# google/automl

Measured on AMD Instinct MI355X. Metric: images/sec EfficientDet-D0 640x640 fwd+bwd (whole job; per-GPU = value / n_gpus), higher is better.
Workload: dtype bf16; 1 GPU; efficientdet-d0 640x640 batch 128/GPU forward+backward+SGD/EMA update (BASELINE configs[2]; DP replicas of it for n_gpus>1); global_batch=128, parallelism=dp1, ranks_seen=1, param_crc32=4110976682, launch=hipGraph replay of the captured step

## Files before the change

automl_amd/csrc/fuse.hip:

```cpp
#include "rowmap_impl.h"

namespace {

constexpr int THREADS = 256;
static_assert(THREADS == ROW_THREADS, "ew_grid sizes its grids for this workgroup size");

struct FuseArgs {
  edet_tview_t in[3];
  int mode[3];
  int pad_t[3], pad_l[3];
  int nin;
  const float* wn;
  int wc;
  int act;
  int n, oh, ow, c, ldo;
  void* gin[3];
  int gbeta[3];
  int write_ds;
  const float* wraw[3];
  float* wn_out;
  int method;
};

__device__ __forceinline__ void normalise_weights(const float (&w)[3], int nin, int method, float (&wn)[3]) {
  if (method == 1) {
    for (int i = 0; i < nin; ++i) wn[i] = 1.f;
    return;
  }
  if (method == 2) {
    float m = w[0], e[3], s = 0.f;
    for (int i = 1; i < nin; ++i) m = fmaxf(m, w[i]);
    for (int i = 0; i < nin; ++i) { e[i] = expf(w[i] - m); s += e[i]; }
    for (int i = 0; i < nin; ++i) wn[i] = e[i] / s;
    return;
  }
  float r[3], s = 0.f;
  for (int i = 0; i < nin; ++i) { r[i] = fmaxf(w[i], 0.f); s += r[i]; }
  for (int i = 0; i < nin; ++i) wn[i] = r[i] / (s + 0.0001f);
}

__device__ __forceinline__ void normalise_weights_bwd(const float (&w)[3], int nin, int method, const float (&dwn)[3],
                                                      float (&dw)[3]) {
  for (int i = 0; i < 3; ++i) dw[i] = 0.f;
  if (method == 1) return;
  if (method == 2) {
    float m = w[0], p[3], s = 0.f, dot = 0.f;
    for (int i = 1; i < nin; ++i) m = fmaxf(m, w[i]);
    for (int i = 0; i < nin; ++i) { p[i] = expf(w[i] - m); s += p[i]; }
    for (int i = 0; i < nin; ++i) { p[i] /= s; dot += dwn[i] * p[i]; }
    for (int i = 0; i < nin; ++i) dw[i] = p[i] * (dwn[i] - dot);
    return;
  }
  float r[3], s = 0.0001f, dot = 0.f;
  for (int i = 0; i < nin; ++i) { r[i] = fmaxf(w[i], 0.f); s += r[i]; }
  for (int i = 0; i < nin; ++i) dot += dwn[i] * r[i];
  for (int i = 0; i < nin; ++i) {
    const float dr = dwn[i] / s - dot / (s * s);
    if (w[i] > 0.f) dw[i] = dr;
  }
}

__device__ __forceinline__ void affine8(const edet_tview_t& v, const ViewCoef& k, float x[8]) {
  if (v.scale) {
#pragma unroll
    for (int e = 0; e < 8; ++e) x[e] = fmaf(x[e], k.scale[e], k.shift[e]);
  }
}

template <typename T, bool ARGMAX>
__device__ __forceinline__ void sample_input(const FuseArgs& a, int i, const ViewCoef& k, int n, int oy,
                                             int ox, int c0, float x[8], uint32_t (&am)[2]) {
  const edet_tview_t& v = a.in[i];
  const T* base = reinterpret_cast<const T*>(v.data);
  if (a.mode[i] == EDET_RS_IDENTITY) {
    load8<T>(base + ((size_t)(n * v.h + oy) * v.w + ox) * v.ld + c0, x);
    affine8(v, k, x);
  } else if (a.mode[i] == EDET_RS_UP2) {
    int sy = a.oh == 2 * v.h ? oy >> 1 : (int)((uint32_t)(oy * v.h) / (uint32_t)a.oh);
    int sx = a.ow == 2 * v.w ? ox >> 1 : (int)((uint32_t)(ox * v.w) / (uint32_t)a.ow);
    sy = sy < v.h - 1 ? sy : v.h - 1;
    sx = sx < v.w - 1 ? sx : v.w - 1;
    load8<T>(base + ((size_t)(n * v.h + sy) * v.w + sx) * v.ld + c0, x);
    affine8(v, k, x);
  } else {
#pragma unroll
    for (int e = 0; e < 8; ++e) x[e] = -INFINITY;
    int idx[8];
#pragma unroll
    for (int e = 0; e < 8; ++e) idx[e] = 0;
    for (int ky = 0; ky < 3; ++ky) {
      const int sy = oy * 2 - a.pad_t[i] + ky;
      if (sy < 0 || sy >= v.h) continue;
      for (int kx = 0; kx < 3; ++kx) {
        const int sx = ox * 2 - a.pad_l[i] + kx;
        if (sx < 0 || sx >= v.w) continue;
        float t[8];
        load8<T>(base + ((size_t)(n * v.h + sy) * v.w + sx) * v.ld + c0, t);
        affine8(v, k, t);
        if (ARGMAX) {
#pragma unroll
          for (int e = 0; e < 8; ++e) {
            const bool gt = t[e] > x[e];
            idx[e] = gt ? ky * 3 + kx : idx[e];
            x[e] = gt ? t[e] : x[e];
          }
        } else {
#pragma unroll
          for (int e = 0; e < 8; ++e) x[e] = fmaxf(x[e], t[e]);
        }
      }
    }
    if (ARGMAX) {
      am[0] = (uint32_t)idx[0] | ((uint32_t)idx[1] << 8) | ((uint32_t)idx[2] << 16) | ((uint32_t)idx[3] << 24);
      am[1] = (uint32_t)idx[4] | ((uint32_t)idx[5] << 8) | ((uint32_t)idx[6] << 16) | ((uint32_t)idx[7] << 24);
    }
  }
}

template <typename T, bool BWD, bool PCDW>
__device__ __forceinline__ void fuse_body(const FuseArgs& a, T* __restrict__ out, const T* __restrict__ dout,
                                          T* __restrict__ ds, float* dwn, unsigned char* __restrict__ pool_argmax,
                                          float* dwn_parts) {
  const int nvec = a.c / 8;
  const int64_t total = (int64_t)a.n * a.oh * a.ow * nvec;
  const bool per_ch = a.wc > 1;
  extern __shared__ float redc[];
  float wn[3] = {0.f, 0.f, 0.f};
  if (!BWD && !per_ch && a.wn_out) {
    float w[3] = {0.f, 0.f, 0.f};
    if (a.method != 1)
      for (int i = 0; i < a.nin; ++i) w[i] = a.wraw[i][0];
    normalise_weights(w, a.nin, a.method, wn);
    if (blockIdx.x == 0 && threadIdx.x < a.nin) a.wn_out[threadIdx.x] = wn[threadIdx.x];
  } else if (!per_ch) {
    for (int i = 0; i < a.nin; ++i) wn[i] = a.wn[i];
  }
  float dw_acc[3] = {0.f, 0.f, 0.f};
  float dwc[PCDW ? 3 : 1][8];
  uint32_t q0 = blockIdx.x * blockDim.x + threadIdx.x, qstride = gridDim.x * blockDim.x;
  const int slices = PCDW ? THREADS / nvec : 1;
  if (PCDW) {
#pragma unroll
    for (int i = 0; i < 3; ++i)
#pragma unroll
      for (int e = 0; e < 8; ++e) dwc[PCDW ? i : 0][e] = 0.f;
    const int chunk = threadIdx.x % nvec, slice = threadIdx.x / nvec;
    q0 = slice < slices ? (uint32_t)((blockIdx.x * slices + slice) * nvec + chunk) : (uint32_t)total;
    qstride = (uint32_t)(gridDim.x * slices * nvec);
  }
  const uint32_t total32 = (uint32_t)total, unvec = (uint32_t)nvec, uow = (uint32_t)a.ow, uoh = (uint32_t)a.oh;
  for (uint32_t q = q0; q < total32; q += qstride) {
    uint32_t pix = q / unvec;
    const int c0 = (int)(q - pix * unvec) * 8;
    const uint32_t prow = pix / uow;
    const int ox = (int)(pix - prow * uow);
    const int n = (int)(prow / uoh);
    const int oy = (int)(prow - (uint32_t)n * uoh);
    float s[8], xi[3][8];
#pragma unroll
    for (int e = 0; e < 8; ++e) s[e] = 0.f;
    const size_t opix = (size_t)(n * a.oh + oy) * a.ow + ox;
    int plane = 0;
    for (int i = 0; i < a.nin; ++i) {
      ViewCoef k;
      view_load_coef(a.in[i], c0, k);
      uint32_t am[2];
      if (BWD && pool_argmax && a.mode[i] == EDET_RS_POOL) {
        sample_input<T, true>(a, i, k, n, oy, ox, c0, xi[i], am);
        *reinterpret_cast<uint2*>(pool_argmax + ((size_t)plane * a.n * a.oh * a.ow + opix) * a.c + c0) =
            make_uint2(am[0], am[1]);
        ++plane;
      } else {
        sample_input<T, false>(a, i, k, n, oy, ox, c0, xi[i], am);
      }
      if (per_ch) {
        float wv[8];
        loadf8(a.wn + (size_t)i * a.wc + c0, wv);
#pragma unroll
        for (int e = 0; e < 8; ++e) s[e] = fmaf(wv[e], xi[i][e], s[e]);
      } else {
#pragma unroll
        for (int e = 0; e < 8; ++e) s[e] = fmaf(wn[i], xi[i][e], s[e]);
      }
    }
    const size_t off = opix * a.ldo + c0;
    if (!BWD) {
      if (a.act == EDET_ACT_SWISH) {
#pragma unroll
        for (int e = 0; e < 8; ++e) s[e] = swishf_(s[e]);
      } else if (a.act > EDET_ACT_SWISH) {
#pragma unroll
        for (int e = 0; e < 8; ++e) s[e] = act_other_(a.act, s[e]);
      }
      store8<T>(out + off, s);
    } else {
      float d[8];
      load8<T>(dout + off, d);
      if (a.act == EDET_ACT_SWISH) {
#pragma unroll
        for (int e = 0; e < 8; ++e) d[e] *= swish_gradf_(s[e]);
      } else if (a.act > EDET_ACT_SWISH) {
#pragma unroll
        for (int e = 0; e < 8; ++e) d[e] *= act_other_grad_(a.act, s[e]);
      }
      if (a.write_ds) store8<T>(ds + off, d);
      for (int i = 0; i < a.nin; ++i) {
        if (a.gin[i]) {
          float g[8];
#pragma unroll
          for (int e = 0; e < 8; ++e) g[e] = to_f<T>(from_f<T>(d[e]));
          if (per_ch) {
            float wv[8];
            loadf8(a.wn + (size_t)i * a.wc + c0, wv);
#pragma unroll
            for (int e = 0; e < 8; ++e) g[e] *= wv[e];
          } else {
#pragma unroll
            for (int e = 0; e < 8; ++e) g[e] *= wn[i];
          }
          T* gp = reinterpret_cast<T*>(a.gin[i]) + opix * a.in[i].ld + c0;
          if (a.gbeta[i]) {
            float old[8];
            load8<T>(gp, old);
#pragma unroll
            for (int e = 0; e < 8; ++e) g[e] += old[e];
          }
          store8<T>(gp, g);
        }
      }
      for (int i = 0; i < a.nin; ++i) {
        if (per_ch) {
          if (PCDW) {
#pragma unroll
// ... 13 lines not shown
#pragma unroll
        for (int e = 0; e < 8; ++e) redc[((size_t)slice * a.nin + i) * a.c + chunk * 8 + e] = dwc[PCDW ? i : 0][e];
    }
    __syncthreads();
    for (int i = threadIdx.x; i < a.nin * a.c; i += THREADS) {
      float t = 0.f;
      for (int sl = 0; sl < slices; ++sl) t += redc[(size_t)sl * a.nin * a.c + i];
      if (dwn_parts) dwn_parts[(size_t)blockIdx.x * a.nin * a.c + i] = t;
      else dwn[i] += t;
    }
  } else if (BWD && dwn && !per_ch) {
    __shared__ float red[THREADS / 64][4];
    for (int i = 0; i < a.nin; ++i) {
      float v = dw_acc[i];
#pragma unroll
      for (int off = 32; off > 0; off >>= 1) v += __shfl_down(v, off, 64);
      if ((threadIdx.x & 63) == 0) red[threadIdx.x >> 6][i] = v;
    }
    __syncthreads();
    if (threadIdx.x < 3) {
      float t = 0.f;
      if (threadIdx.x < a.nin)
        for (int w = 0; w < THREADS / 64; ++w) t += red[w][threadIdx.x];
      if (dwn_parts) dwn_parts[(size_t)blockIdx.x * 4 + threadIdx.x] = t;
      else if (threadIdx.x < a.nin) dwn[threadIdx.x] += t;
    }
  }
}

template <typename T, bool BWD>
__global__ __launch_bounds__(THREADS) void k_fuse(const FuseArgs a, T* __restrict__ out,
                                                 const T* __restrict__ dout, T* __restrict__ ds,
                                                 float* dwn, unsigned char* __restrict__ pool_argmax,
                                                 float* dwn_parts = nullptr) {
  fuse_body<T, BWD, false>(a, out, dout, ds, dwn, pool_argmax, dwn_parts);
}
template <typename T>
__global__ __launch_bounds__(THREADS) void k_fuse_pc(const FuseArgs a, T* __restrict__ out,
                                                    const T* __restrict__ dout, T* __restrict__ ds,
                                                    float* dwn, unsigned char* __restrict__ pool_argmax,
                                                    float* dwn_parts) {
  fuse_body<T, true, true>(a, out, dout, ds, dwn, pool_argmax, dwn_parts);
}

struct FuseWBwd {
  const float* w[3];
  float* dw[3];
  int nin, method;
};
__global__ __launch_bounds__(256) void k_fuse_dwn_finish(const float* __restrict__ parts, int G, float* dwn, FuseWBwd wb) {
  __shared__ float red[256][3];
  __shared__ float tot[3];
  float t[3] = {0.f, 0.f, 0.f};
  const int per = (G + 255) / 256;
  for (int g = threadIdx.x * per; g < min(G, (threadIdx.x + 1) * per); ++g)
    for (int i = 0; i < 3; ++i) t[i] += parts[(size_t)g * 4 + i];
  for (int i = 0; i < 3; ++i) red[threadIdx.x][i] = t[i];
  __syncthreads();
  if (threadIdx.x < 3) {
    float s = 0.f;
    for (int q = 0; q < 256; ++q) s += red[q][threadIdx.x];
    dwn[threadIdx.x] += s;
    tot[threadIdx.x] = dwn[threadIdx.x];
  }
  if (wb.nin == 0 || wb.method == 1) return;
  __syncthreads();
  if (threadIdx.x == 0) {
    float w[3] = {0.f, 0.f, 0.f}, d[3] = {tot[0], tot[1], tot[2]}, dw[3];
    for (int i = 0; i < wb.nin; ++i) w[i] = wb.w[i][0];
    normalise_weights_bwd(w, wb.nin, wb.method, d, dw);
    for (int i = 0; i < wb.nin; ++i)
      if (wb.method == 2 || w[i] > 0.f) wb.dw[i][0] += dw[i];
  }
}

struct FuseInArgs {
  edet_tview_t in;
  int mode, pad_t, pad_l;
  const float* wn;
  int wc;
  int idx;
  int n, oh, ow, ldds;
  int beta;
};

template <typename T>
__global__ __launch_bounds__(THREADS) void k_fuse_bwd_input(const FuseInArgs a, const T* __restrict__ ds,
                                                           T* __restrict__ gout,
                                                           const unsigned char* __restrict__ argmax) {
  const edet_tview_t& v = a.in;
  const int nvec = v.c / 8;
  const int64_t total = (int64_t)v.n * v.h * v.w * nvec;
  const float wn = a.wc > 1 ? 0.f : a.wn[a.idx];
  const T* base = reinterpret_cast<const T*>(v.data);
  const uint32_t total32 = (uint32_t)total, unvec = (uint32_t)nvec, uw = (uint32_t)v.w, uh = (uint32_t)v.h;
  for (uint32_t q = blockIdx.x * blockDim.x + threadIdx.x; q < total32; q += gridDim.x * blockDim.x) {
    const uint32_t pix = q / unvec;
    const int c0 = (int)(q - pix * unvec) * 8;
    const uint32_t prow = pix / uw;
    const int sx = (int)(pix - prow * uw);
    const int n = (int)(prow / uh);
    const int sy = (int)(prow - (uint32_t)n * uh);
    float g[8];
#pragma unroll
    for (int e = 0; e < 8; ++e) g[e] = 0.f;
    if (a.mode == EDET_RS_IDENTITY) {
      load8<T>(ds + ((size_t)(n * a.oh + sy) * a.ow + sx) * a.ldds + c0, g);
    } else if (a.mode == EDET_RS_UP2) {
      const bool x2 = a.oh == 2 * v.h && a.ow == 2 * v.w;
      const int oy_lo = x2 ? 2 * sy : (int)(((uint32_t)(sy * a.oh) + uh - 1) / uh);
      int oy_hi = x2 ? 2 * sy + 2 : (int)(((uint32_t)((sy + 1) * a.oh) + uh - 1) / uh);
      const int ox_lo = x2 ? 2 * sx : (int)(((uint32_t)(sx * a.ow) + uw - 1) / uw);
      int ox_hi = x2 ? 2 * sx + 2 : (int)(((uint32_t)((sx + 1) * a.ow) + uw - 1) / uw);
      if (sy == v.h - 1) oy_hi = a.oh;
      if (sx == v.w - 1) ox_hi = a.ow;
      for (int oy = oy_lo; oy < oy_hi; ++oy)
        for (int ox = ox_lo; ox < ox_hi; ++ox) {
          float t[8];
          load8<T>(ds + ((size_t)(n * a.oh + oy) * a.ow + ox) * a.ldds + c0, t);
#pragma unroll
          for (int e = 0; e < 8; ++e) g[e] += t[e];
        }
    } else if (argmax) {
      for (int oy = (sy + a.pad_t - 2 + 1) / 2; oy <= (sy + a.pad_t) / 2; ++oy) {
        if (oy < 0 || oy >= a.oh) continue;
        for (int ox = (sx + a.pad_l - 2 + 1) / 2; ox <= (sx + a.pad_l) / 2; ++ox) {
          if (ox < 0 || ox >= a.ow) continue;
          const uint32_t tap = (uint32_t)((sy - (oy * 2 - a.pad_t)) * 3 + (sx - (ox * 2 - a.pad_l)));
          const size_t opix = (size_t)(n * a.oh + oy) * a.ow + ox;
          const uint2 am = *reinterpret_cast<const uint2*>(argmax + opix * v.c + c0);
          float t[8];
          load8<T>(ds + opix * a.ldds + c0, t);
#pragma unroll
          for (int e = 0; e < 8; ++e) {
            const uint32_t w = e < 4 ? am.x : am.y;
            if (((w >> (8 * (e & 3))) & 0xffu) == tap) g[e] += t[e];
          }
        }
      }
    } else {
      ViewCoef k;
      view_load_coef(v, c0, k);
      float mine[8];
      load8<T>(base + ((size_t)(n * v.h + sy) * v.w + sx) * v.ld + c0, mine);
      affine8(v, k, mine);
      for (int oy = (sy + a.pad_t - 2 + 1) / 2; oy <= (sy + a.pad_t) / 2; ++oy) {
        if (oy < 0 || oy >= a.oh) continue;
        for (int ox = (sx + a.pad_l - 2 + 1) / 2; ox <= (sx + a.pad_l) / 2; ++ox) {
          if (ox < 0 || ox >= a.ow) continue;
          bool win[8];
#pragma unroll
          for (int e = 0; e < 8; ++e) win[e] = true;
          for (int ky = 0; ky < 3; ++ky) {
            const int yy = oy * 2 - a.pad_t + ky;
            if (yy < 0 || yy >= v.h) continue;
            for (int kx = 0; kx < 3; ++kx) {
              const int xx = ox * 2 - a.pad_l + kx;
              if (xx < 0 || xx >= v.w) continue;
              if (yy == sy && xx == sx) continue;
              float t[8];
              load8<T>(base + ((size_t)(n * v.h + yy) * v.w + xx) * v.ld + c0, t);
              affine8(v, k, t);
              const bool before = (yy < sy) || (yy == sy && xx < sx);
#pragma unroll
              for (int e = 0; e < 8; ++e) {
                if (before ? (t[e] >= mine[e]) : (t[e] > mine[e])) win[e] = false;
              }
            }
          }
          float t[8];
          load8<T>(ds + ((size_t)(n * a.oh + oy) * a.ow + ox) * a.ldds + c0, t);
#pragma unroll
          for (int e = 0; e < 8; ++e)
            if (win[e]) g[e] += t[e];
        }
      }
    }
    const size_t off = ((size_t)(n * v.h + sy) * v.w + sx) * v.ld + c0;
    if (a.wc > 1) {
      float wv[8];
      loadf8(a.wn + (size_t)a.idx * a.wc + c0, wv);
#pragma unroll
      for (int e = 0; e < 8; ++e) g[e] *= wv[e];
    } else {
#pragma unroll
      for (int e = 0; e < 8; ++e) g[e] *= wn;
    }
    if (a.beta) {
      float old[8];
      load8<T>(gout + off, old);
#pragma unroll
      for (int e = 0; e < 8; ++e) g[e] += old[e];
    }
    store8<T>(gout + off, g);
  }
}

__global__ void k_fuse_weights(const float* w0, const float* w1, const float* w2, int nin, int method,
                               float* wn, int wc) {
  const int ch = blockIdx.x * blockDim.x + threadIdx.x;
  if (ch >= wc) return;
  const float* wp[3] = {w0, w1, w2};
  float w[3] = {0.f, 0.f, 0.f}, r[3];
  if (method != 1)
    for (int i = 0; i < nin; ++i) w[i] = wp[i][ch];
  normalise_weights(w, nin, method, r);
  for (int i = 0; i < nin; ++i) wn[i * wc + ch] = r[i];
}

__global__ void k_fuse_weights_bwd(const float* w0, const float* w1, const float* w2, int nin, int method,
                                   const float* dwn, float* dw0, float* dw1, float* dw2, int wc) {
  const int ch = blockIdx.x * blockDim.x + threadIdx.x;
  if (ch >= wc || method == 1) return;
  const float* wp[3] = {w0, w1, w2};
  float* dwp[3] = {dw0, dw1, dw2};
  float w[3] = {0.f, 0.f, 0.f}, d[3] = {0.f, 0.f, 0.f}, dw[3];
  for (int i = 0; i < nin; ++i) { w[i] = wp[i][ch]; d[i] = dwn[i * wc + ch]; }
  normalise_weights_bwd(w, nin, method, d, dw);
  for (int i = 0; i < nin; ++i)
    if (method == 2 || w[i] > 0.f) dwp[i][ch] += dw[i];
}

int fill_args(FuseArgs& a, const edet_tview_t* in0, const edet_tview_t* in1, const edet_tview_t* in2,
              const int* modes, int nin, const float* wn, int wc, int act, int oh, int ow, int ldo) {
  EDET_CHECK(nin >= 1 && nin <= 3 && in0 && modes && wn, "edet_fuse: bad arguments");
  EDET_CHECK(wc == 1 || wc == in0->c, "edet_fuse: wc must be 1 or the channel count (got %d)", wc);
  const edet_tview_t* ins[3] = {in0, in1, in2};
  memset(&a, 0, sizeof(a));
  a.nin = nin; a.wn = wn; a.wc = wc; a.act = act; a.oh = oh; a.ow = ow; a.ldo = ldo;
  for (int i = 0; i < nin; ++i) {
    EDET_CHECK(ins[i] && ins[i]->data, "edet_fuse: null input %d", i);
    a.in[i] = *ins[i];
    a.mode[i] = modes[i];
    EDET_CHECK(ins[i]->act == EDET_ACT_NONE && !ins[i]->gate, "edet_fuse: inputs must be affine-only views");
    EDET_CHECK(ins[i]->c == in0->c && ins[i]->n == in0->n && ins[i]->c % 8 == 0 && ins[i]->ld % 8 == 0,
               "edet_fuse: channel/batch mismatch");
    if (modes[i] == EDET_RS_IDENTITY) {
      EDET_CHECK(ins[i]->h == oh && ins[i]->w == ow, "edet_fuse: identity input %d has a different size", i);
    } else if (modes[i] == EDET_RS_UP2) {
      EDET_CHECK(ins[i]->h <= oh && ins[i]->w <= ow, "edet_fuse: upsample input %d is larger than the output", i);
    } else if (modes[i] == EDET_RS_POOL) {
      EDET_CHECK(same_out(ins[i]->h, 2) == oh && same_out(ins[i]->w, 2) == ow,
                 "Incompatible Resampling : feat shape %dx%d target_shape: %dx%d", ins[i]->h, ins[i]->w, oh, ow);
      a.pad_t[i] = same_pad_before(ins[i]->h, 3, 2);
      a.pad_l[i] = same_pad_before(ins[i]->w, 3, 2);
    } else {
      EDET_CHECK(false, "edet_fuse: bad mode %d", modes[i]);
    }
  }
  a.n = in0->n; a.c = in0->c;
  EDET_CHECK(ldo % 8 == 0 && ldo >= a.c, "edet_fuse: bad ldo");
  return 0;
}

}

extern "C" int edet_fuse_weights(const float* w0, const float* w1, const float* w2, int nin,
                                 int method, float* wn, int wc, void* stream) {
  EDET_CHECK(wn && (method == 1 || w0) && wc >= 1, "edet_fuse_weights: bad arguments");
  edet_launch(k_fuse_weights, dim3((wc + 63) / 64), dim3(64), 0, to_stream(stream), w0, w1, w2, nin, method, wn, wc);
  EDET_LAUNCH_CHECK("edet_fuse_weights");
  return 0;
}

extern "C" int edet_fuse_weights_bwd(const float* w0, const float* w1, const float* w2, int nin,
                                     int method, const float* dwn, float* dw0, float* dw1, float* dw2,
                                     int wc, void* stream) {
  if (method == 1) return 0;
  EDET_CHECK(w0 && dwn && dw0 && wc >= 1, "edet_fuse_weights_bwd: bad arguments");
  edet_launch(k_fuse_weights_bwd, dim3((wc + 63) / 64), dim3(64), 0, to_stream(stream), w0, w1, w2, nin, method, dwn, dw0, dw1, dw2, wc);
  EDET_LAUNCH_CHECK("edet_fuse_weights_bwd");
  return 0;
}

extern "C" int edet_fuse_fwd(const edet_tview_t* in0, const edet_tview_t* in1, const edet_tview_t* in2,
                             const int* modes, int nin, float* wn, int wc, int act,
                             void* out, int oh, int ow, int ldo, const float* const* wraw, int method, int dtype,
                             void* stream) {
  FuseArgs a;
  if (int rc = fill_args(a, in0, in1, in2, modes, nin, wn, wc, act, oh, ow, ldo)) return rc;
  EDET_CHECK(out, "edet_fuse_fwd: null output");
  if (wraw && wc == 1) {
    EDET_CHECK(method >= 0 && method <= 2, "edet_fuse_fwd: bad method %d", method);
    for (int i = 0; i < nin; ++i) {
      EDET_CHECK(method == 1 || wraw[i], "edet_fuse_fwd: null fusion variable %d", i);
      a.wraw[i] = wraw[i];
    }
    a.wn_out = wn;
    a.method = method;
  }
  EDET_CHECK((int64_t)a.n * oh * ow * (a.c / 8) < (1ll << 31), "edet_fuse_fwd: tensor too large for the 32-bit index arithmetic");
  const int grid = ew_grid((int64_t)a.n * oh * ow * (a.c / 8), dtype == EDET_BF16 ? reinterpret_cast<const void*>(&k_fuse<bf16_t, false>) : nullptr);
  if (dtype == EDET_BF16) edet_launch(k_fuse<bf16_t, false>, grid, dim3(THREADS), 0, to_stream(stream), a, (bf16_t*)out, nullptr, nullptr, nullptr, nullptr, nullptr);
  else if (dtype == EDET_F32) edet_launch(k_fuse<float, false>, grid, dim3(THREADS), 0, to_stream(stream), a, (float*)out, nullptr, nullptr, nullptr, nullptr, nullptr);
  else EDET_CHECK(false, "edet_fuse_fwd: bad dtype %d", dtype);
  EDET_LAUNCH_CHECK("edet_fuse_fwd");
  return 0;
}

extern "C" int edet_fuse_bwd_pre(const edet_tview_t* in0, const edet_tview_t* in1, const edet_tview_t* in2,
                                 const int* modes, int nin, const float* wn, int wc, int act,
                                 const void* dout, int oh, int ow, int ldo,
                                 void* ds, float* dwn, void* pool_argmax, void* const* gin, const int* gbeta,
                                 int write_ds, void* workspace, size_t workspace_bytes, const float* const* wraw,
                                 int method, float* const* dwraw, int dtype, void* stream) {
  FuseArgs a;
  if (int rc = fill_args(a, in0, in1, in2, modes, nin, wn, wc, act, oh, ow, ldo)) return rc;
  EDET_CHECK(dout && ds, "edet_fuse_bwd_pre: null pointer");
  a.write_ds = write_ds;
  for (int i = 0; i < nin; ++i) {
    a.gin[i] = gin ? gin[i] : nullptr;
    a.gbeta[i] = (gin && gbeta) ? gbeta[i] : 0;
    EDET_CHECK(!a.gin[i] || modes[i] == EDET_RS_IDENTITY, "edet_fuse_bwd_pre: gin[%d] given for a resampled input", i);
  }
  const bool pcdw = wc > 1 && dwn;
  EDET_CHECK(!pcdw || a.c <= 8 * THREADS, "edet_fuse_bwd_pre: per-channel fusion weights need c <= %d", 8 * THREADS);
  const size_t lds = pcdw ? (size_t)(THREADS / (a.c / 8)) * nin * a.c * sizeof(float) : 0;
  EDET_CHECK((int64_t)a.n * oh * ow * (a.c / 8) < (1ll << 31), "edet_fuse_bwd_pre: tensor too large for the 32-bit index arithmetic");
  int grid = ew_grid((int64_t)a.n * oh * ow * (a.c / 8), dtype == EDET_BF16 ? (pcdw ? reinterpret_cast<const void*>(&k_fuse_pc<bf16_t>) : reinterpret_cast<const void*>(&k_fuse<bf16_t, true>)) : nullptr, lds);
  const size_t row = pcdw ? (size_t)nin * a.c : 4;
  float* parts = (dwn && workspace && workspace_bytes >= (size_t)grid * row * sizeof(float)) ? reinterpret_cast<float*>(workspace) : nullptr;
  if (dwn && !parts) grid = 1;
  if (pcdw) {
    if (dtype == EDET_BF16) edet_launch(k_fuse_pc<bf16_t>, grid, dim3(THREADS), lds, to_stream(stream), a, nullptr, (const bf16_t*)dout, (bf16_t*)ds, dwn, (unsigned char*)pool_argmax, parts);
    else if (dtype == EDET_F32) edet_launch(k_fuse_pc<float>, grid, dim3(THREADS), lds, to_stream(stream), a, nullptr, (const float*)dout, (float*)ds, dwn, (unsigned char*)pool_argmax, parts);
    else EDET_CHECK(false, "edet_fuse_bwd_pre: bad dtype %d", dtype);
    EDET_LAUNCH_CHECK("edet_fuse_bwd_pre");
    if (parts && edet_reduce_partials2(parts, grid, (int64_t)nin * a.c, dwn, (int64_t)nin * a.c, nullptr, to_stream(stream)) != 0) return -2;
    return 0;
  }
  if (dtype == EDET_BF16) edet_launch(k_fuse<bf16_t, true>, grid, dim3(THREADS), lds, to_stream(stream), a, nullptr, (const bf16_t*)dout, (bf16_t*)ds, dwn, (unsigned char*)pool_argmax, parts);
  else if (dtype == EDET_F32) edet_launch(k_fuse<float, true>, grid, dim3(THREADS), lds, to_stream(stream), a, nullptr, (const float*)dout, (float*)ds, dwn, (unsigned char*)pool_argmax, parts);
  else EDET_CHECK(false, "edet_fuse_bwd_pre: bad dtype %d", dtype);
  if (parts) {
    FuseWBwd wb;
    memset(&wb, 0, sizeof(wb));
    if (wraw && dwraw && method != 1) {
      EDET_CHECK(method == 0 || method == 2, "edet_fuse_bwd_pre: bad method %d", method);
      for (int i = 0; i < nin; ++i) {
        EDET_CHECK(wraw[i] && dwraw[i], "edet_fuse_bwd_pre: null fusion variable %d", i);
        wb.w[i] = wraw[i];
        wb.dw[i] = dwraw[i];
      }
      wb.nin = nin;
      wb.method = method;
    }
    edet_launch(k_fuse_dwn_finish, dim3(1), dim3(256), 0, to_stream(stream), (const float*)parts, grid, dwn, wb);
  } else {
    EDET_CHECK(!(wraw && dwraw) || method == 1, "edet_fuse_bwd_pre: the fusion variables' gradient needs wc == 1 and a workspace of %zu bytes",
               (size_t)grid * 4 * sizeof(float));
  }
  EDET_LAUNCH_CHECK("edet_fuse_bwd_pre");
  return 0;
}

extern "C" int edet_fuse_bwd_input(const edet_tview_t* in, int mode, const float* wn, int wc, int idx,
                                   const void* ds, int oh, int ow, int lds_, const void* pool_argmax,
                                   void* gout, int beta, int dtype, void* stream) {
  EDET_CHECK(in && in->data && wn && ds && gout && idx >= 0 && idx < 3, "edet_fuse_bwd_input: bad arguments");
  EDET_CHECK(in->c % 8 == 0 && in->ld % 8 == 0 && lds_ % 8 == 0, "edet_fuse_bwd_input: c/ld % 8");
  EDET_CHECK(wc == 1 || wc == in->c, "edet_fuse_bwd_input: wc must be 1 or the channel count (got %d)", wc);
  FuseInArgs a;
  memset(&a, 0, sizeof(a));
  a.in = *in; a.mode = mode; a.wn = wn; a.wc = wc; a.idx = idx; a.n = in->n; a.oh = oh; a.ow = ow; a.ldds = lds_;
  a.beta = beta;
  if (mode == EDET_RS_POOL) {
    a.pad_t = same_pad_before(in->h, 3, 2);
    a.pad_l = same_pad_before(in->w, 3, 2);
  }
  EDET_CHECK((int64_t)in->n * in->h * in->w * (in->c / 8) < (1ll << 31), "edet_fuse_bwd_input: tensor too large for the 32-bit index arithmetic");
  const int grid = ew_grid((int64_t)in->n * in->h * in->w * (in->c / 8), dtype == EDET_BF16 ? reinterpret_cast<const void*>(&k_fuse_bwd_input<bf16_t>) : nullptr);
  const unsigned char* am = mode == EDET_RS_POOL ? reinterpret_cast<const unsigned char*>(pool_argmax) : nullptr;
  if (dtype == EDET_BF16) edet_launch(k_fuse_bwd_input<bf16_t>, grid, dim3(THREADS), 0, to_stream(stream), a, (const bf16_t*)ds, (bf16_t*)gout, am);
  else if (dtype == EDET_F32) edet_launch(k_fuse_bwd_input<float>, grid, dim3(THREADS), 0, to_stream(stream), a, (const float*)ds, (float*)gout, am);
  else EDET_CHECK(false, "edet_fuse_bwd_input: bad dtype %d", dtype);
  EDET_LAUNCH_CHECK("edet_fuse_bwd_input");
  return 0;
}
```

automl_amd/engine.py:

```python
import ctypes

import torch

from automl_amd import _lib
from automl_amd import netspec as netspec_lib
from automl_amd._lib import ACT_NONE, ACT_SWISH, EDET_BF16, RS_IDENTITY, RS_POOL, RS_UP2, call, ptr
from automl_amd.layer_engine import BN, LayerEngine, ParamArena, Raw, Update, View, capture_graph


class Engine(LayerEngine):

  def __init__(self, config, batch_size, image_size=None, dtype='bf16', device='cuda:0', seed=0,
               params=None, spec=None, stochastic_depth=True, arena=None):
    self.config = config
    momentum = float(config.momentum)
    adam = str(config.optimizer).lower() == 'adam'
    super().__init__(spec if spec is not None else netspec_lib.NetSpec(config), batch_size,
                     image_size if image_size is not None else config.image_size, dtype=dtype, device=device, seed=seed,
                     params=params, arena=arena, stochastic_depth=stochastic_depth,
                     update=Update('adam', momentum, self.ADAM_BETA2, self.ADAM_EPSILON) if adam else Update('sgd', momentum))
    if adam:
      self.arena.second_moment()
    self._side = None
    self.small_level_stream = True
    self._side_pending = False
    self.loss_sums = self.zbuf('loss_sums', (4,))
    self.pool_argmax = True
    self._overlap_reduce = None
    self._reduce_marks = {}
    self._comm_stream = None
    self._bucket_no = 0

  def _side_branch(self):
    if self._side is None:
      names = [n for n in self.seg_names if n.startswith('class_net/') or n.startswith('box_net/')]
      lo = min(self.offsets[n][0] for n in names)
      hi = max(self.offsets[n][0] + self.offsets[n][1] for n in names)
      self._side_range = (lo, hi)
      self._side_grads = torch.zeros(self.n_train_elems, dtype=torch.float32, device=self.device)
      self._side = self._new_branch(torch.cuda.Stream(device=self.device), self._side_grads)
    return self._side

  def _fork_join(self, main_job, side_job):
    side = self._side_branch()
    main = torch.cuda.current_stream(self.device)
    rec = _lib.recorder
    fork = torch.cuda.Event()
    fork.record(main)
    side.stream.wait_event(fork)
    if rec is not None:
      rec.stream_wait(side.stream.cuda_stream, rec.event_record(main.cuda_stream))
    try:
      self._branch = side
      with torch.cuda.stream(side.stream):
        b = side_job()
        done = torch.cuda.Event()
        done.record(side.stream)
        rec_done = rec.event_record(side.stream.cuda_stream) if rec is not None else None
      self._branch = self._main
      a = main_job()
    finally:
      self._branch = self._main
    main.wait_event(done)
    if rec is not None:
      rec.stream_wait(main.cuda_stream, rec_done)
    return a, b

  def _join_side(self):
    if self._side_pending:
      lo, hi = self._side_range
      call('edet_axpy_clear', self.grads_flat.data_ptr() + 4 * lo, self._side_grads.data_ptr() + 4 * lo, hi - lo, 1,
           self.stream)
      self._side_pending = False

  def fuse(self, key, inputs, modes, wnames, oh, ow, act=ACT_SWISH):
    c = inputs[0].raw.c
    n = inputs[0].raw.n
    nin = len(inputs)
    out = Raw(self, key, n, oh, ow, c)
    wm = self.spec.fpn.weight_method
    wc = c if (wnames and wm.startswith('channel_')) else 1
    wn = self.buf(key + ':wn', (max(4, 3 * wc),), torch.float32)
    method = (2 if wm in ('attn', 'channel_attn') else 0) if wnames else 1
    wp = [ptr(self.param(w)) for w in wnames] + [None] * (3 - len(wnames)) if wnames else [None] * 3
    wfold = wc == 1
    wraw = (ctypes.c_void_p * 3)(*wp) if wfold else None
    if not wfold:
      call('edet_fuse_weights', wp[0], wp[1], wp[2], nin, method, ptr(wn), wc, self.stream)
    tv = [v.tview() for v in inputs]
    tvp = [ctypes.byref(t) for t in tv] + [None] * (3 - nin)
    marr = (ctypes.c_int * 3)(*(list(modes) + [0] * (3 - nin)))
    fbytes = (sum(v.raw.rows for v in inputs) + out.rows) * c * self.esize
    call('edet_fuse_fwd', tvp[0], tvp[1], tvp[2], marr, nin, ptr(wn), wc, act, ptr(out.data), oh, ow, out.ld,
         wraw, method, self.dtype, self.stream, nbytes=fbytes)
    vout = View(out)
    for v in inputs:
      v.consumers += 1
    if self.training:
      ds = self.buf(key + ':ds', (n, oh, ow, out.ld), self.tdtype)
      dwn = self.zbuf(key + ':dwn', (max(4, 3 * wc),))
      npool = sum(1 for m in modes if m == RS_POOL)
      amax = self.buf(key + ':amax', (npool, n, oh, ow, c), torch.uint8) if npool and self.pool_argmax else None

      def bwd():
        assert out.grad_written, key
        tv2 = [v.tview() for v in inputs]
        tvp2 = [ctypes.byref(t) for t in tv2] + [None] * (3 - nin)
        merged = [modes[i] == RS_IDENTITY and v.raw.needs_grad for i, v in enumerate(inputs)]
        gin = (ctypes.c_void_p * 3)()
        gbeta = (ctypes.c_int * 3)()
        for i, v in enumerate(inputs):
          if merged[i]:
            gin[i] = ptr(v.raw.ensure_grad())
            gbeta[i] = 1 if v.raw.grad_written else 0
            v.raw.grad_written = True
        write_ds = 1 if any(v.raw.needs_grad and not merged[i] for i, v in enumerate(inputs)) else 0
        wgrad_folded = wfold and bool(wnames) and method != 1
        dwraw = (ctypes.c_void_p * 3)(*([ptr(self.grad(w)) for w in wnames] + [None] * (3 - len(wnames)))) if wgrad_folded else None
        call('edet_fuse_bwd_pre', tvp2[0], tvp2[1], tvp2[2], marr, nin, ptr(wn), wc, act, ptr(out.grad), oh, ow,
             out.ld, ptr(ds), ptr(dwn), ptr(amax), gin, gbeta, write_ds, *self._ws(),
             wraw if wgrad_folded else None, method, dwraw, self.dtype, self.stream,
             nbytes=fbytes + out.rows * c * self.esize)
        plane = 0
        for i, v in enumerate(inputs):
          am = None
          if modes[i] == RS_POOL and amax is not None:
            am = amax[plane].data_ptr()
            plane += 1
          if not v.raw.needs_grad or merged[i]:
            continue
          g = v.raw.ensure_grad()
          call('edet_fuse_bwd_input', ctypes.byref(tv2[i]), modes[i], ptr(wn), wc, i, ptr(ds), oh, ow, out.ld, am,
               ptr(g), 1 if v.raw.grad_written else 0, self.dtype, self.stream,
               nbytes=(out.rows + v.raw.rows) * c * self.esize,
               tag='%dx%dx%d %s' % (v.raw.h, v.raw.w, c, ('id', 'up2', 'pool')[modes[i]]))
          v.raw.grad_written = True
        if wnames and not wgrad_folded:
          gp = [ptr(self.grad(w)) for w in wnames] + [None] * (3 - len(wnames))
          call('edet_fuse_weights_bwd', wp[0], wp[1], wp[2], nin, method, ptr(dwn), gp[0], gp[1], gp[2],
               wc, self.stream)

      self.tape.append(bwd)
    return vout

  def forward(self, images, training=False, update_moving=True):
    c = self.config
    spec = self.spec
    self._begin(training, update_moving)
    if training and self.drop_masks and not torch.cuda.is_current_stream_capturing():
      self.refresh_drop_masks()
    bb = c.backbone_name
    x = self.stem(bb, images, self.act)
    reds = []
    self._reduce_marks = {}
    bucket_blocks = self._bucket_blocks() if (training and self._overlap_reduce is not None) else ()
    for b in spec.blocks:
      if b.index in bucket_blocks:
        self._reduce_marks[len(self.tape)] = bucket_blocks[b.index]
      x = self._mbconv(x, b, '%s/blocks_%d' % (bb, b.index))
      if b.index in spec.reductions:
        reds.append(x)
    all_feats = [None] + reds
    feats = list(all_feats[c.min_level:c.max_level + 1])
    wf = c.fpn_num_filters
    if training and self._overlap_reduce is not None:
      self._reduce_marks[0] = 0
      self._reduce_marks[len(self.tape)] = self._first_non_backbone_elem()
    for level in range(6, c.max_level + 1):
      f = feats[-1]
      th, tw = (f.raw.h + 1) // 2, (f.raw.w + 1) // 2
      s = 'resample_p%d' % level
      if f.raw.c != wf and getattr(c, 'conv_after_downsample', False):
        pooled = self.fuse(s + ':pool', [f], [RS_POOL], [], th, tw, act=ACT_NONE)
        feats.append(self.pw(s, pooled, s + '/conv2d/kernel', wf, bias=s + '/conv2d/bias', bn=(s + '/bn') if c.apply_bn_for_resampling else None, bias_grad=True))
        continue
      if f.raw.c != wf:
        f = self.pw(s, f, s + '/conv2d/kernel', wf, bias=s + '/conv2d/bias', bn=(s + '/bn') if c.apply_bn_for_resampling else None, bias_grad=True)
      feats.append(self.fuse(s + ':pool', [f], [RS_POOL], [], th, tw, act=ACT_NONE))
    for rep in range(c.fpn_cell_repeats):
      feats = self._fpn_cell(feats, 'fpn_cells/cell_%d' % rep)
    self.fpn_feats = feats
    na = spec.num_anchors
    nbig = sum(1 for f in feats if f.raw.h * f.raw.w > 400)
    if self.small_level_stream and self.sync_bn is None and 0 < nbig < len(feats):
      cls, box = self._heads_two_chains(feats, nbig, c.num_classes * na, 4 * na)
    else:
      cls = self._head(feats, 'class_net', 'class', c.num_classes * na)
      box = self._head(feats, 'box_net', 'box', 4 * na)
    self.cls_views, self.box_views = cls, box
    if self._cast_items and not torch.cuda.is_current_stream_capturing() and \
        (self._cast_table is None or self._cast_table[0] != list(self._cast_items)):
      self._cast_all()
    return cls, box

  def _fpn_cell(self, feats, cell_scope):
    c = self.config
    wf = c.fpn_num_filters
    fpn = self.spec.fpn
    feats = list(feats)
# ... 301 lines not shown
```

Before: 2886 images/sec.

## Add specialized BiFPN fuse fast paths and merge up2 input gradient into fused backward

Adds templated fast paths for the common BiFPN fusion patterns (identity+upsample2, identity+pool, identity+identity+pool). They batch raw vector loads ahead of the math, hoist the per-channel affine coefficients, and unroll over several grid strides. In backward, the upsampled input's gradient is now computed inside the pre-kernel by iterating over coarse pixels and summing their four fine children. This removes the separate bwd_input launch and the ds buffer write/read for that case. It also adds dedicated up2 and pool-argmax paths in the standalone input-gradient kernel, at the cost of more template instantiations and register pressure.

```diff
diff --git a/automl_amd/csrc/fuse.hip b/automl_amd/csrc/fuse.hip
--- a/automl_amd/csrc/fuse.hip
+++ b/automl_amd/csrc/fuse.hip
@@ -20,6 +20,28 @@
   const float* wraw[3];
   float* wn_out;
   int method;
+  int fast;
+};
+
+enum { FUSE_GENERIC = 0, FUSE_ID_UP2 = 1, FUSE_ID_ID_POOL = 2, FUSE_ID_POOL = 3, FUSE_ID_UP2_QUAD = 4 };
+constexpr int FUSE_DEPTH_UP2 = 2, FUSE_DEPTH_POOL = 1;
+
+template <typename T> struct Raw8;
+template <> struct Raw8<bf16_t> {
+  uint4 v;
+  __device__ __forceinline__ void load(const bf16_t* p) { v = *reinterpret_cast<const uint4*>(p); }
+  __device__ __forceinline__ void get(float x[8]) const { unpack8(v, x); }
+};
+template <> struct Raw8<float> {
+  float4 a, b;
+  __device__ __forceinline__ void load(const float* p) {
+    a = *reinterpret_cast<const float4*>(p);
+    b = *reinterpret_cast<const float4*>(p + 4);
+  }
+  __device__ __forceinline__ void get(float x[8]) const {
+    x[0] = a.x; x[1] = a.y; x[2] = a.z; x[3] = a.w;
+    x[4] = b.x; x[5] = b.y; x[6] = b.z; x[7] = b.w;
+  }
 };
 
 __device__ __forceinline__ void normalise_weights(const float (&w)[3], int nin, int method, float (&wn)[3]) {
@@ -114,6 +136,269 @@
       am[0] = (uint32_t)idx[0] | ((uint32_t)idx[1] << 8) | ((uint32_t)idx[2] << 16) | ((uint32_t)idx[3] << 24);
       am[1] = (uint32_t)idx[4] | ((uint32_t)idx[5] << 8) | ((uint32_t)idx[6] << 16) | ((uint32_t)idx[7] << 24);
     }
+  }
+}
+
+template <typename T, bool BWD, int NIN, int LAST, int UU>
+__device__ __forceinline__ void fuse_fast_trip(const FuseArgs& a, T* __restrict__ out, const T* __restrict__ dout,
+                                               T* __restrict__ ds, unsigned char* __restrict__ pool_argmax,
+                                               const float (&wn)[3], ViewCoef (&k)[NIN], bool hoisted, uint32_t q,
+                                               uint32_t qstride, float (&dw_acc)[3]) {
+  constexpr int NID = NIN - 1, NTAP = LAST == EDET_RS_POOL ? 9 : 1;
+  const uint32_t unvec = (uint32_t)(a.c / 8), uow = (uint32_t)a.ow, uoh = (uint32_t)a.oh;
+  const edet_tview_t& vl = a.in[NID];
+  int c0[UU];
+  size_t opix[UU];
+  uint32_t inside[UU];
+  Raw8<T> rid[UU][NID], rlast[UU][NTAP], rd[UU], rold[UU][NID];
+#pragma unroll
+  for (int u = 0; u < UU; ++u) {
+    const uint32_t qq = q + (uint32_t)u * qstride;
+    const uint32_t pix = qq / unvec;
+    c0[u] = (int)(qq - pix * unvec) * 8;
+    const uint32_t prow = pix / uow;
+    const int ox = (int)(pix - prow * uow);
+    const int n = (int)(prow / uoh);
+    const int oy = (int)(prow - (uint32_t)n * uoh);
+    opix[u] = (size_t)(n * a.oh + oy) * a.ow + ox;
+#pragma unroll
+    for (int i = 0; i < NID; ++i)
+      rid[u][i].load(reinterpret_cast<const T*>(a.in[i].data) + opix[u] * a.in[i].ld + c0[u]);
+    const T* base = reinterpret_cast<const T*>(vl.data);
+    inside[u] = 0;
+    if (LAST == EDET_RS_UP2) {
+      rlast[u][0].load(base + ((size_t)(n * vl.h + (oy >> 1)) * vl.w + (ox >> 1)) * vl.ld + c0[u]);
+    } else {
+#pragma unroll
+      for (int ky = 0; ky < 3; ++ky) {
+        const int sy = oy * 2 - a.pad_t[NID] + ky;
+        const int cy = min(max(sy, 0), vl.h - 1);
+#pragma unroll
+        for (int kx = 0; kx < 3; ++kx) {
+          const int sx = ox * 2 - a.pad_l[NID] + kx;
+          const int cx = min(max(sx, 0), vl.w - 1);
+          inside[u] |= (sy == cy && sx == cx) ? 1u << (ky * 3 + kx) : 0u;
+          rlast[u][NTAP == 9 ? ky * 3 + kx : 0].load(base + ((size_t)(n * vl.h + cy) * vl.w + cx) * vl.ld + c0[u]);
+        }
+      }
+    }
+    if (BWD) {
+      rd[u].load(dout + opix[u] * a.ldo + c0[u]);
+#pragma unroll
+      for (int i = 0; i < NID; ++i)
+        if (a.gin[i] && a.gbeta[i])
+          rold[u][i].load(reinterpret_cast<const T*>(a.gin[i]) + opix[u] * a.in[i].ld + c0[u]);
+    }
+  }
+#pragma unroll
+  for (int u = 0; u < UU; ++u) {
+    if (!hoisted) {
+#pragma unroll
+      for (int i = 0; i < NIN; ++i) view_load_coef(a.in[i], c0[u], k[i]);
+    }
+    float s[8], xi[NIN][8];
+#pragma unroll
+    for (int e = 0; e < 8; ++e) s[e] = 0.f;
+#pragma unroll
+    for (int i = 0; i < NID; ++i) {
+      rid[u][i].get(xi[i]);
+      affine8(a.in[i], k[i], xi[i]);
+#pragma unroll
+      for (int e = 0; e < 8; ++e) s[e] = fmaf(wn[i], xi[i][e], s[e]);
+    }
+    if (LAST == EDET_RS_UP2) {
+      rlast[u][0].get(xi[NID]);
+      affine8(vl, k[NID], xi[NID]);
+    } else {
+      int idx[8];
+#pragma unroll
+      for (int e = 0; e < 8; ++e) { xi[NID][e] = -INFINITY; idx[e] = 0; }
+#pragma unroll
+      for (int tap = 0; tap < NTAP; ++tap) {
+        float t[8];
+        rlast[u][tap].get(t);
+        affine8(vl, k[NID], t);
+        const bool in = (inside[u] >> tap) & 1u;
+#pragma unroll
+        for (int e = 0; e < 8; ++e) {
+          t[e] = in ? t[e] : -INFINITY;
+          if (BWD) {
+            const bool gt = t[e] > xi[NID][e];
+            idx[e] = gt ? tap : idx[e];
+            xi[NID][e] = gt ? t[e] : xi[NID][e];
+          } else {
+            xi[NID][e] = fmaxf(xi[NID][e], t[e]);
+          }
+        }
+      }
+      if (BWD)
+        *reinterpret_cast<uint2*>(pool_argmax + opix[u] * a.c + c0[u]) =
+            make_uint2((uint32_t)idx[0] | ((uint32_t)idx[1] << 8) | ((uint32_t)idx[2] << 16) | ((uint32_t)idx[3] << 24),
+                       (uint32_t)idx[4] | ((uint32_t)idx[5] << 8) | ((uint32_t)idx[6] << 16) | ((uint32_t)idx[7] << 24));
+    }
+#pragma unroll
+    for (int e = 0; e < 8; ++e) s[e] = fmaf(wn[NID], xi[NID][e], s[e]);
+    const size_t off = opix[u] * a.ldo + c0[u];
+    if (!BWD) {
+      if (a.act == EDET_ACT_SWISH) {
+#pragma unroll
+        for (int e = 0; e < 8; ++e) s[e] = swishf_(s[e]);
+      } else if (a.act > EDET_ACT_SWISH) {
+#pragma unroll
+        for (int e = 0; e < 8; ++e) s[e] = act_other_(a.act, s[e]);
+      }
+      store8<T>(out + off, s);
+    } else {
+      float d[8];
+      rd[u].get(d);
+      if (a.act == EDET_ACT_SWISH) {
+#pragma unroll
+        for (int e = 0; e < 8; ++e) d[e] *= swish_gradf_(s[e]);
+      } else if (a.act > EDET_ACT_SWISH) {
+#pragma unroll
+        for (int e = 0; e < 8; ++e) d[e] *= act_other_grad_(a.act, s[e]);
+      }
+      if (a.write_ds) store8<T>(ds + off, d);
+#pragma unroll
+      for (int i = 0; i < NID; ++i) {
+        if (a.gin[i]) {
+#pragma clang fp contract(off)
+          float g[8];
+#pragma unroll
+          for (int e = 0; e < 8; ++e) g[e] = to_f<T>(from_f<T>(d[e]));
+#pragma unroll
+          for (int e = 0; e < 8; ++e) g[e] *= wn[i];
+          if (a.gbeta[i]) {
+            float old[8];
+            rold[u][i].get(old);
+#pragma unroll
+            for (int e = 0; e < 8; ++e) g[e] += old[e];
+          }
+          store8<T>(reinterpret_cast<T*>(a.gin[i]) + opix[u] * a.in[i].ld + c0[u], g);
+        }
+      }
+#pragma unroll
+      for (int i = 0; i < NIN; ++i)
+#pragma unroll
+        for (int e = 0; e < 8; ++e) dw_acc[i] = fmaf(d[e], xi[i][e], dw_acc[i]);
+    }
+  }
+}
+
+template <typename T, bool BWD, int NIN, int LAST>
+__device__ __forceinline__ void fuse_fast_loop(const FuseArgs& a, T* __restrict__ out, const T* __restrict__ dout,
+                                               T* __restrict__ ds, unsigned char* __restrict__ pool_argmax,
+                                               const float (&wn)[3], uint32_t q0, uint32_t qstride, uint32_t total32,
+                                               float (&dw_acc)[3]) {
+  const uint32_t unvec = (uint32_t)(a.c / 8);
+  const bool hoisted = qstride % unvec == 0;
+  ViewCoef k[NIN];
+  if (hoisted) {
+#pragma unroll
+    for (int i = 0; i < NIN; ++i) view_load_coef(a.in[i], (int)(q0 % unvec) * 8, k[i]);
+  }
+  constexpr int DEPTH = LAST == EDET_RS_POOL ? FUSE_DEPTH_POOL : FUSE_DEPTH_UP2;
+  uint32_t q = q0;
+  for (; q + (DEPTH - 1) * qstride < total32; q += DEPTH * qstride)
+    fuse_fast_trip<T, BWD, NIN, LAST, DEPTH>(a, out, dout, ds, pool_argmax, wn, k, hoisted, q, qstride, dw_acc);
+  for (; q < total32; q += qstride)
+    fuse_fast_trip<T, BWD, NIN, LAST, 1>(a, out, dout, ds, pool_argmax, wn, k, hoisted, q, qstride, dw_acc);
+}
+
+
+template <typename T>
+__device__ __forceinline__ void fuse_up2_quad_loop(const FuseArgs& a, const T* __restrict__ dout, T* __restrict__ ds,
+                                                   const float (&wn)[3], uint32_t q0, uint32_t qstride,
+                                                   float (&dw_acc)[3]) {
+  const edet_tview_t& vc = a.in[1];
+  const uint32_t unvec = (uint32_t)(a.c / 8), uw = (uint32_t)vc.w, uh = (uint32_t)vc.h;
+  const uint32_t total32 = (uint32_t)a.n * uh * uw * unvec;
+  const bool hoisted = qstride % unvec == 0;
+  ViewCoef k[2];
+  if (hoisted) {
+#pragma unroll
+    for (int i = 0; i < 2; ++i) view_load_coef(a.in[i], (int)(q0 % unvec) * 8, k[i]);
+  }
+  const bool old0 = a.gin[0] && a.gbeta[0], old1 = a.gbeta[1] != 0;
+  for (uint32_t q = q0; q < total32; q += qstride) {
+    const uint32_t pix = q / unvec;
+    const int c0 = (int)(q - pix * unvec) * 8;
+    const uint32_t prow = pix / uw;
+    const int sx = (int)(pix - prow * uw);
+    const int n = (int)(prow / uh);
+    const int sy = (int)(prow - (uint32_t)n * uh);
+    const size_t cpix = (size_t)(n * vc.h + sy) * vc.w + sx;
+    size_t opix[4];
+    Raw8<T> rc, rid[4], rd[4], rold0[4], rold1;
+    rc.load(reinterpret_cast<const T*>(vc.data) + cpix * vc.ld + c0);
+#pragma unroll
+    for (int j = 0; j < 4; ++j) {
+      opix[j] = (size_t)(n * a.oh + 2 * sy + (j >> 1)) * a.ow + 2 * sx + (j & 1);
+      rid[j].load(reinterpret_cast<const T*>(a.in[0].data) + opix[j] * a.in[0].ld + c0);
+      rd[j].load(dout + opix[j] * a.ldo + c0);
+      if (old0) rold0[j].load(reinterpret_cast<const T*>(a.gin[0]) + opix[j] * a.in[0].ld + c0);
+    }
+    if (old1) rold1.load(reinterpret_cast<const T*>(a.gin[1]) + cpix * vc.ld + c0);
+    if (!hoisted) {
+#pragma unroll
+      for (int i = 0; i < 2; ++i) view_load_coef(a.in[i], c0, k[i]);
+    }
+    float xc[8], gc[8];
+    rc.get(xc);
+    affine8(vc, k[1], xc);
+#pragma unroll
+    for (int e = 0; e < 8; ++e) gc[e] = 0.f;
+#pragma unroll
+    for (int j = 0; j < 4; ++j) {
+      float s[8], x0[8], d[8];
+      rid[j].get(x0);
+      affine8(a.in[0], k[0], x0);
+#pragma unroll
+      for (int e = 0; e < 8; ++e) s[e] = fmaf(wn[1], xc[e], fmaf(wn[0], x0[e], 0.f));
+      rd[j].get(d);
+      if (a.act == EDET_ACT_SWISH) {
+#pragma unroll
+        for (int e = 0; e < 8; ++e) d[e] *= swish_gradf_(s[e]);
+      } else if (a.act > EDET_ACT_SWISH) {
+#pragma unroll
+        for (int e = 0; e < 8; ++e) d[e] *= act_other_grad_(a.act, s[e]);
+      }
+      if (a.write_ds) store8<T>(ds + opix[j] * a.ldo + c0, d);
+      float r[8];
+#pragma unroll
+      for (int e = 0; e < 8; ++e) r[e] = to_f<T>(from_f<T>(d[e]));
+#pragma unroll
+      for (int e = 0; e < 8; ++e) gc[e] += r[e];
+      if (a.gin[0]) {
+#pragma clang fp contract(off)
+        float g[8];
+#pragma unroll
+        for (int e = 0; e < 8; ++e) g[e] = r[e] * wn[0];
+        if (old0) {
+          float old[8];
+          rold0[j].get(old);
+#pragma unroll
+          for (int e = 0; e < 8; ++e) g[e] += old[e];
+        }
+        store8<T>(reinterpret_cast<T*>(a.gin[0]) + opix[j] * a.in[0].ld + c0, g);
+      }
+#pragma unroll
+      for (int e = 0; e < 8; ++e) dw_acc[0] = fmaf(d[e], x0[e], dw_acc[0]);
+#pragma unroll
+      for (int e = 0; e < 8; ++e) dw_acc[1] = fmaf(d[e], xc[e], dw_acc[1]);
+    }
+    {
+#pragma clang fp contract(off)
+#pragma unroll
+      for (int e = 0; e < 8; ++e) gc[e] *= wn[1];
+      if (old1) {
+        float old[8];
+        rold1.get(old);
+#pragma unroll
+        for (int e = 0; e < 8; ++e) gc[e] += old[e];
+      }
+    }
+    store8<T>(reinterpret_cast<T*>(a.gin[1]) + cpix * vc.ld + c0, gc);
   }
 }
 
@@ -149,6 +434,17 @@
     qstride = (uint32_t)(gridDim.x * slices * nvec);
   }
   const uint32_t total32 = (uint32_t)total, unvec = (uint32_t)nvec, uow = (uint32_t)a.ow, uoh = (uint32_t)a.oh;
+  if (!PCDW && a.fast != FUSE_GENERIC) {
+    if (BWD && a.fast == FUSE_ID_UP2_QUAD)
+      fuse_up2_quad_loop<T>(a, dout, ds, wn, q0, qstride, dw_acc);
+    else if (a.fast == FUSE_ID_UP2)
+      fuse_fast_loop<T, BWD, 2, EDET_RS_UP2>(a, out, dout, ds, pool_argmax, wn, q0, qstride, total32, dw_acc);
+    else if (a.fast == FUSE_ID_ID_POOL)
+      fuse_fast_loop<T, BWD, 3, EDET_RS_POOL>(a, out, dout, ds, pool_argmax, wn, q0, qstride, total32, dw_acc);
+    else
+      fuse_fast_loop<T, BWD, 2, EDET_RS_POOL>(a, out, dout, ds, pool_argmax, wn, q0, qstride, total32, dw_acc);
+    q0 = total32;
+  }
   for (uint32_t q = q0; q < total32; q += qstride) {
     uint32_t pix = q / unvec;
     const int c0 = (int)(q - pix * unvec) * 8;
@@ -328,7 +624,9 @@
   int idx;
   int n, oh, ow, ldds;
   int beta;
+  int fast;
 };
+enum { FUSE_IN_GENERIC = 0, FUSE_IN_UP2 = 1, FUSE_IN_POOL_ARGMAX = 2 };
 
 template <typename T>
 __global__ __launch_bounds__(THREADS) void k_fuse_bwd_input(const FuseInArgs a, const T* __restrict__ ds,
@@ -350,6 +648,54 @@
     float g[8];
 #pragma unroll
     for (int e = 0; e < 8; ++e) g[e] = 0.f;
+    const size_t goff = ((size_t)(n * v.h + sy) * v.w + sx) * v.ld + c0;
+    if (a.fast != FUSE_IN_GENERIC) {
+#pragma clang fp contract(off)
+      const bool pool = a.fast == FUSE_IN_POOL_ARGMAX;
+      int oy[2], ox[2];
+      bool oky[2], okx[2];
+      if (pool) {
+        oy[0] = (sy + a.pad_t - 2 + 1) / 2; oy[1] = (sy + a.pad_t) / 2;
+        ox[0] = (sx + a.pad_l - 2 + 1) / 2; ox[1] = (sx + a.pad_l) / 2;
+        oky[0] = oy[0] < a.oh; oky[1] = oy[1] != oy[0] && oy[1] < a.oh;
+        okx[0] = ox[0] < a.ow; okx[1] = ox[1] != ox[0] && ox[1] < a.ow;
+      } else {
+        oy[0] = 2 * sy; oy[1] = 2 * sy + 1;
+        ox[0] = 2 * sx; ox[1] = 2 * sx + 1;
+        oky[0] = oky[1] = okx[0] = okx[1] = true;
+      }
+      Raw8<T> rt[4], rold;
+      uint2 am[4];
+#pragma unroll
+      for (int j = 0; j < 4; ++j) {
+        const size_t opix = (size_t)(n * a.oh + min(oy[j >> 1], a.oh - 1)) * a.ow + min(ox[j & 1], a.ow - 1);
+        rt[j].load(ds + opix * a.ldds + c0);
+        am[j] = pool ? *reinterpret_cast<const uint2*>(argmax + opix * v.c + c0) : make_uint2(0u, 0u);
+      }
+      if (a.beta) rold.load(gout + goff);
+#pragma unroll
+      for (int j = 0; j < 4; ++j) {
+        float t[8];
+        rt[j].get(t);
+        const bool ok = oky[j >> 1] && okx[j & 1];
+        const uint32_t tap = (uint32_t)((sy - (oy[j >> 1] * 2 - a.pad_t)) * 3 + (sx - (ox[j & 1] * 2 - a.pad_l)));
+#pragma unroll
+        for (int e = 0; e < 8; ++e) {
+          const uint32_t w = e < 4 ? am[j].x : am[j].y;
+          if (ok && (!pool || ((w >> (8 * (e & 3))) & 0xffu) == tap)) g[e] += t[e];
+        }
+      }
+#pragma unroll
+      for (int e = 0; e < 8; ++e) g[e] *= wn;
+      if (a.beta) {
+        float old[8];
+        rold.get(old);
+#pragma unroll
+        for (int e = 0; e < 8; ++e) g[e] += old[e];
+      }
+      store8<T>(gout + goff, g);
+      continue;
+    }
     if (a.mode == EDET_RS_IDENTITY) {
       load8<T>(ds + ((size_t)(n * a.oh + sy) * a.ow + sx) * a.ldds + c0, g);
     } else if (a.mode == EDET_RS_UP2) {
@@ -496,6 +842,14 @@
   }
   a.n = in0->n; a.c = in0->c;
   EDET_CHECK(ldo % 8 == 0 && ldo >= a.c, "edet_fuse: bad ldo");
+  a.fast = FUSE_GENERIC;
+  bool ids = wc == 1 && nin >= 2;
+  for (int i = 0; i + 1 < nin; ++i) ids = ids && modes[i] == EDET_RS_IDENTITY;
+  if (ids) {
+    const edet_tview_t* last = ins[nin - 1];
+    if (modes[nin - 1] == EDET_RS_UP2 && nin == 2 && oh == 2 * last->h && ow == 2 * last->w) a.fast = FUSE_ID_UP2;
+    else if (modes[nin - 1] == EDET_RS_POOL) a.fast = nin == 3 ? FUSE_ID_ID_POOL : FUSE_ID_POOL;
+  }
   return 0;
 }
 
@@ -552,18 +906,23 @@
                                  int method, float* const* dwraw, int dtype, void* stream) {
   FuseArgs a;
   if (int rc = fill_args(a, in0, in1, in2, modes, nin, wn, wc, act, oh, ow, ldo)) return rc;
-  EDET_CHECK(dout && ds, "edet_fuse_bwd_pre: null pointer");
+  EDET_CHECK(dout && (ds || !write_ds), "edet_fuse_bwd_pre: null pointer");
   a.write_ds = write_ds;
   for (int i = 0; i < nin; ++i) {
     a.gin[i] = gin ? gin[i] : nullptr;
     a.gbeta[i] = (gin && gbeta) ? gbeta[i] : 0;
-    EDET_CHECK(!a.gin[i] || modes[i] == EDET_RS_IDENTITY, "edet_fuse_bwd_pre: gin[%d] given for a resampled input", i);
-  }
+    EDET_CHECK(!a.gin[i] || modes[i] == EDET_RS_IDENTITY || (i == 1 && a.fast == FUSE_ID_UP2),
+               "edet_fuse_bwd_pre: gin[%d] given for a resampled input", i);
+  }
+  const bool quad = a.fast == FUSE_ID_UP2 && a.gin[1];
+  if (quad) a.fast = FUSE_ID_UP2_QUAD;
+  const int64_t items = quad ? (int64_t)a.n * a.in[1].h * a.in[1].w * (a.c / 8) : (int64_t)a.n * oh * ow * (a.c / 8);
+  if (!pool_argmax && (a.fast == FUSE_ID_ID_POOL || a.fast == FUSE_ID_POOL)) a.fast = FUSE_GENERIC;
   const bool pcdw = wc > 1 && dwn;
   EDET_CHECK(!pcdw || a.c <= 8 * THREADS, "edet_fuse_bwd_pre: per-channel fusion weights need c <= %d", 8 * THREADS);
   const size_t lds = pcdw ? (size_t)(THREADS / (a.c / 8)) * nin * a.c * sizeof(float) : 0;
   EDET_CHECK((int64_t)a.n * oh * ow * (a.c / 8) < (1ll << 31), "edet_fuse_bwd_pre: tensor too large for the 32-bit index arithmetic");
-  int grid = ew_grid((int64_t)a.n * oh * ow * (a.c / 8), dtype == EDET_BF16 ? (pcdw ? reinterpret_cast<const void*>(&k_fuse_pc<bf16_t>) : reinterpret_cast<const void*>(&k_fuse<bf16_t, true>)) : nullptr, lds);
+  int grid = ew_grid(items, dtype == EDET_BF16 ? (pcdw ? reinterpret_cast<const void*>(&k_fuse_pc<bf16_t>) : reinterpret_cast<const void*>(&k_fuse<bf16_t, true>)) : nullptr, lds);
   const size_t row = pcdw ? (size_t)nin * a.c : 4;
   float* parts = (dwn && workspace && workspace_bytes >= (size_t)grid * row * sizeof(float)) ? reinterpret_cast<float*>(workspace) : nullptr;
   if (dwn && !parts) grid = 1;
@@ -617,6 +976,8 @@
   EDET_CHECK((int64_t)in->n * in->h * in->w * (in->c / 8) < (1ll << 31), "edet_fuse_bwd_input: tensor too large for the 32-bit index arithmetic");
   const int grid = ew_grid((int64_t)in->n * in->h * in->w * (in->c / 8), dtype == EDET_BF16 ? reinterpret_cast<const void*>(&k_fuse_bwd_input<bf16_t>) : nullptr);
   const unsigned char* am = mode == EDET_RS_POOL ? reinterpret_cast<const unsigned char*>(pool_argmax) : nullptr;
+  if (wc == 1 && mode == EDET_RS_UP2 && oh == 2 * in->h && ow == 2 * in->w) a.fast = FUSE_IN_UP2;
+  else if (wc == 1 && mode == EDET_RS_POOL && am) a.fast = FUSE_IN_POOL_ARGMAX;
   if (dtype == EDET_BF16) edet_launch(k_fuse_bwd_input<bf16_t>, grid, dim3(THREADS), 0, to_stream(stream), a, (const bf16_t*)ds, (bf16_t*)gout, am);
   else if (dtype == EDET_F32) edet_launch(k_fuse_bwd_input<float>, grid, dim3(THREADS), 0, to_stream(stream), a, (const float*)ds, (float*)gout, am);
   else EDET_CHECK(false, "edet_fuse_bwd_input: bad dtype %d", dtype);
diff --git a/automl_amd/engine.py b/automl_amd/engine.py
--- a/automl_amd/engine.py
+++ b/automl_amd/engine.py
@@ -97,7 +97,6 @@
     for v in inputs:
       v.consumers += 1
     if self.training:
-      ds = self.buf(key + ':ds', (n, oh, ow, out.ld), self.tdtype)
       dwn = self.zbuf(key + ':dwn', (max(4, 3 * wc),))
       npool = sum(1 for m in modes if m == RS_POOL)
       amax = self.buf(key + ':amax', (npool, n, oh, ow, c), torch.uint8) if npool and self.pool_argmax else None
@@ -106,7 +105,10 @@
         assert out.grad_written, key
         tv2 = [v.tview() for v in inputs]
         tvp2 = [ctypes.byref(t) for t in tv2] + [None] * (3 - nin)
-        merged = [modes[i] == RS_IDENTITY and v.raw.needs_grad for i, v in enumerate(inputs)]
+        up2_merged = (wc == 1 and list(modes) == [RS_IDENTITY, RS_UP2] and
+                      oh == 2 * inputs[1].raw.h and ow == 2 * inputs[1].raw.w)
+        merged = [(modes[i] == RS_IDENTITY or (i == 1 and up2_merged)) and v.raw.needs_grad
+                  for i, v in enumerate(inputs)]
         gin = (ctypes.c_void_p * 3)()
         gbeta = (ctypes.c_int * 3)()
         for i, v in enumerate(inputs):
@@ -115,6 +117,7 @@
             gbeta[i] = 1 if v.raw.grad_written else 0
             v.raw.grad_written = True
         write_ds = 1 if any(v.raw.needs_grad and not merged[i] for i, v in enumerate(inputs)) else 0
+        ds = self.buf(key + ':ds', (n, oh, ow, out.ld), self.tdtype) if write_ds else None
         wgrad_folded = wfold and bool(wnames) and method != 1
         dwraw = (ctypes.c_void_p * 3)(*([ptr(self.grad(w)) for w in wnames] + [None] * (3 - len(wnames)))) if wgrad_folded else None
         call('edet_fuse_bwd_pre', tvp2[0], tvp2[1], tvp2[2], marr, nin, ptr(wn), wc, act, ptr(out.grad), oh, ow,
```

New measurement: 2946 images/sec (median of 6 runs). 2.1% higher.
